# akhilmurthy/spacedrive

Hardware: AMD Instinct MI355X
Metric: cas_id files/sec + BLAKE3 GB/s hashed (node) at 1/2/4/8 MI355X (higher is better)
Workload: dtype u32

## Files before the change

### include/sdcas.h

```cpp
#ifndef SDCAS_H
#define SDCAS_H

#include <stddef.h>
#include <stdint.h>

#ifdef __cplusplus
extern "C" {
#endif

#define SDCAS_OK 0
#define SDCAS_E_NO_DEVICE (-1)
#define SDCAS_E_INVALID (-2)
#define SDCAS_E_OOM (-3)
#define SDCAS_E_HIP (-4)
#define SDCAS_E_CAPACITY (-5)
#define SDCAS_E_CANCELLED (-6)

#define SDCAS_STATUS_UNEXPECTED_EOF 100001
#define SDCAS_STATUS_CANCELLED 125

#define SDCAS_MAX_BATCH 0x7FFFFFFF

#define SDCAS_SAMPLE_COUNT 4
#define SDCAS_SAMPLE_SIZE 10240
// ... 284 lines not shown
int sdcas_dev_dedup_combine_async(sdcas_ctx *ctx, const uint64_t *d_keys, const uint8_t *d_has_key,
                                  const int32_t *d_status, const uint64_t *d_ids, size_t n, uint32_t world,
                                  uint64_t *d_rec, uint32_t *d_slot, uint32_t *d_starts, void *stream);
int sdcas_dev_dedup_resolve(sdcas_ctx *ctx, const uint64_t *d_frec, size_t nf, const uint64_t *d_erec,
                            size_t ne, int64_t *d_result, void *stream);
int sdcas_dev_dedup_apply(sdcas_ctx *ctx, const uint64_t *d_ids, const uint32_t *d_slot, size_t n,
                          const int64_t *d_result, size_t chunk_size, const uint64_t *d_plan, int64_t *d_link,
                          uint64_t *d_counts, void *stream);
int sdcas_dev_dedup_combine_buckets(sdcas_ctx *ctx, const uint64_t *d_keys, const uint8_t *d_has_key,
                                    const int32_t *d_status, const uint64_t *d_ids, size_t n, uint32_t world,
                                    size_t cap, uint64_t *d_send, uint32_t *d_slot, int64_t *d_counts,
                                    uint32_t *d_overflow, void *stream);
int sdcas_dev_dedup_resolve_buckets(sdcas_ctx *ctx, const uint64_t *d_frec, size_t fcap, const int64_t *d_fcounts,
                                    const uint64_t *d_erec, size_t ecap, const int64_t *d_ecounts, uint32_t world,
                                    int64_t *d_result, void *stream);
int sdcas_dev_dedup_local(sdcas_ctx *ctx, const uint64_t *d_keys, const uint8_t *d_has_key,
                          const int32_t *d_status, const uint64_t *d_ids, size_t n, const uint64_t *d_ekeys,
                          const uint64_t *d_eids, size_t ne, size_t chunk_size, uint64_t n_total,
                          uint64_t max_steps, uint32_t more, int64_t *d_link, uint64_t *d_counts,
                          uint64_t *d_plan_header, void *stream);

typedef struct sdcas_node sdcas_node;
int sdcas_node_init(const int32_t *devices, size_t n_devices, const sdcas_options *opts, sdcas_node **out_node);
void sdcas_node_destroy(sdcas_node *node);
const char *sdcas_node_last_error(const sdcas_node *node);
size_t sdcas_node_size(const sdcas_node *node);
int sdcas_node_uses_rccl(const sdcas_node *node);
int sdcas_node_set_progress(sdcas_node *node, sdcas_progress_fn progress, void *user, const volatile int32_t *cancel);
int sdcas_node_cas_ids(sdcas_node *node, const char *const *paths, const uint64_t *sizes, size_t n,
                       uint64_t *out_keys, int32_t *out_status);
// ... 15 lines not shown
```

### spacedrive_amd/csrc/b3_batch.h

```cpp
#pragma once
#include <hip/hip_runtime.h>
#include <stddef.h>
#include <stdint.h>

namespace sdcas {

constexpr uint32_t kTile = 1024;
constexpr uint32_t kWG = 512;
constexpr uint32_t kSmallTile = 128;
constexpr uint64_t kSmallSlots = 1ull << 14;
constexpr int kSmallVariant = 84;
constexpr uint32_t kSortTotalsWords = 256;
constexpr uint32_t kSortPerWG = 4096;
inline size_t sort_key_words(size_t max_msgs) { return kSortTotalsWords + 256 * (max_msgs / kSortPerWG + 1); }

struct BatchWorkspace {
  uint64_t* S = nullptr;
  uint32_t* tile_first = nullptr;
  uint64_t* total = nullptr;
  uint32_t* nodes = nullptr;
  void* scan_tmp = nullptr;
  size_t scan_tmp_bytes = 0;
  uint32_t cap_msgs = 0;
  uint64_t cap_chunks = 0;
  uint64_t cap_slots = 0;
  int variant = -1;
  uint64_t small_slots = kSmallSlots;
  int small_variant = kSmallVariant;
  uint64_t cap_small_tiles = 0;
// ... 79 lines not shown
```

### spacedrive_amd/csrc/b3_batch.hip

```cpp
#include <hip/hip_runtime.h>

#include <atomic>
#ifdef SDCAS_ABLATIONS
#include <hipcub/hipcub.hpp>
#endif
#include <stdint.h>
#include <cstdio>
#include <cstring>

#include "b3_device.h"
#include "b3_batch.h"
#include "b3_tree.h"

namespace sdcas {

using namespace b3d;

constexpr int kMaxStack = 64;
constexpr int kMaxStackBig = 64;


template <uint32_t TILE = kTile>
__global__ void k_tile_first(const uint64_t* __restrict__ lens, const uint64_t* __restrict__ S, uint32_t n,
                             uint64_t cap_chunks, uint32_t* __restrict__ tile_first, uint64_t* __restrict__ total) {
// ... 928 lines not shown
                       dim3(kFinishQWG), 0, st, lens, n, S, tile_first, total, cap_slots, nodes, perm, out32,
                       out_keys);
  else
    hipLaunchKernelGGL(k_finish_t<TILE>, dim3((uint32_t)((tiles + kFinishWG - 1) / kFinishWG)), dim3(kFinishWG), 0,
                       st, lens, n, S, tile_first, total, cap_slots, nodes, perm, out32, out_keys);
}

#ifdef SDCAS_ABLATIONS
#include "b3_ablate_kernels.inc"
#endif

constexpr uint32_t kShapeBins = 256;
constexpr uint32_t kScatterPerWG = 4096;
constexpr uint32_t kScatterR = kScatterPerWG / 256;
constexpr uint32_t kShapeManyChunks = 15 << 4;
static_assert(kSortTotalsWords == kShapeBins && kSortPerWG == kScatterPerWG, "ws.sort_keys layout");

__device__ __forceinline__ uint32_t shape_key(uint64_t L) {
  const uint64_t C = chunk_count(L);
  const uint64_t last = L - (C - 1) * CHUNK_LEN;
  const uint32_t blocks = last == 0 ? 1u : (uint32_t)((last + BLOCK_LEN - 1) / BLOCK_LEN);
  return ((uint32_t)min<uint64_t>(C, 15) << 4) | (blocks - 1);
}

__global__ void __launch_bounds__(256) k_shape_hist(const uint64_t* __restrict__ lens, uint32_t n,
                                                    uint32_t* __restrict__ wcnt) {
  __shared__ uint32_t h[kShapeBins];
  const uint32_t t = threadIdx.x;
  h[t] = 0;
  __syncthreads();
  const uint64_t lo = (uint64_t)blockIdx.x * kScatterPerWG;
  uint64_t L[kScatterR];
#pragma unroll
  for (uint32_t r = 0; r < kScatterR; ++r) {
    const uint64_t i = lo + r * 256 + t;
    L[r] = i < n ? lens[i] : 0;
  }
#pragma unroll
  for (uint32_t r = 0; r < kScatterR; ++r)
    if (lo + r * 256 + t < n) atomicAdd(&h[shape_key(L[r])], 1u);
  __syncthreads();
  wcnt[(uint64_t)t * gridDim.x + blockIdx.x] = h[t];
}

__global__ void __launch_bounds__(256) k_shape_bins(uint32_t* __restrict__ wcnt, uint32_t nwg,
                                                    uint32_t* __restrict__ totals) {
  __shared__ uint32_t ws[4];
  __shared__ uint32_t carry;
  const uint32_t t = threadIdx.x, lane = t & 63, wave = t >> 6;
  uint32_t* col = wcnt + (uint64_t)blockIdx.x * nwg;
  if (t == 0) carry = 0;
  __syncthreads();
  for (uint32_t base = 0; base < nwg; base += 256) {
    const uint32_t i = base + t;
    const uint32_t v = i < nwg ? col[i] : 0u;
    uint32_t inc = v;
#pragma unroll
    for (uint32_t d = 1; d < 64; d <<= 1) {
      const uint32_t x = __shfl_up(inc, d);
      if (lane >= d) inc += x;
    }
    if (lane == 63) ws[wave] = inc;
    __syncthreads();
    uint32_t before = carry;
    for (uint32_t w = 0; w < wave; ++w) before += ws[w];
    if (i < nwg) col[i] = before + inc - v;
    __syncthreads();
    if (t == 255) carry = before + inc;
    __syncthreads();
  }
  if (t == 0) totals[blockIdx.x] = carry;
}

__global__ void __launch_bounds__(256) k_shape_scatter(const uint64_t* __restrict__ offs,
                                                       const uint64_t* __restrict__ lens, uint32_t n,
                                                       const uint32_t* __restrict__ totals,
                                                       const uint32_t* __restrict__ wstart,
                                                       uint32_t* __restrict__ perm, uint64_t* __restrict__ soffs,
                                                       uint64_t* __restrict__ slens) {
  __shared__ uint32_t gstart[kShapeBins], lstart[kShapeBins], h[kShapeBins];
  __shared__ uint16_t order[kScatterPerWG];
  __shared__ uint8_t keyof[kScatterPerWG];
  __shared__ uint32_t few_chunks;
  const uint32_t t = threadIdx.x;
  const uint32_t bin_count = totals[t];
  gstart[t] = bin_count;
  h[t] = 0;
  __syncthreads();
  for (uint32_t d = 1; d < kShapeBins; d <<= 1) {
    const uint32_t v = t >= d ? gstart[t - d] : 0u;
    __syncthreads();
    gstart[t] += v;
    __syncthreads();
  }
  if (t == kShapeManyChunks - 1) few_chunks = gstart[t];
  const uint32_t excl = gstart[t] - bin_count;
  __syncthreads();
  gstart[t] = excl;
  const uint32_t lo = blockIdx.x * kScatterPerWG, hi = min(n, lo + kScatterPerWG), m = hi - lo;
  if ((uint64_t)(n - few_chunks) * 10 > (uint64_t)n * 6) {
    uint64_t o[kScatterR], l[kScatterR];
#pragma unroll
    for (uint32_t r = 0; r < kScatterR; ++r) {
      const uint32_t k = t + r * 256;
      o[r] = k < m ? offs[lo + k] : 0;
      l[r] = k < m ? lens[lo + k] : 0;
    }
#pragma unroll
    for (uint32_t r = 0; r < kScatterR; ++r) {
      const uint32_t k = t + r * 256;
      if (k >= m) continue;
      perm[lo + k] = lo + k;
      soffs[lo + k] = o[r];
      slens[lo + k] = l[r];
    }
    return;
  }
  {
    uint64_t l[kScatterR];
#pragma unroll
    for (uint32_t r = 0; r < kScatterR; ++r) {
      const uint32_t k = t + r * 256;
      l[r] = k < m ? lens[lo + k] : 0;
    }
#pragma unroll
    for (uint32_t r = 0; r < kScatterR; ++r) {
      const uint32_t k = t + r * 256;
      if (k >= m) continue;
      const uint32_t key = shape_key(l[r]);
      keyof[k] = (uint8_t)key;
      atomicAdd(&h[key], 1u);
    }
  }
  __syncthreads();
  const uint32_t cnt = h[t];
  gstart[t] += wstart[(uint64_t)t * gridDim.x + blockIdx.x];
  lstart[t] = cnt;
  __syncthreads();
  for (uint32_t d = 1; d < kShapeBins; d <<= 1) {
    const uint32_t v = t >= d ? lstart[t - d] : 0u;
    __syncthreads();
    lstart[t] += v;
    __syncthreads();
  }
  lstart[t] -= cnt;
  h[t] = 0;
  __syncthreads();
  for (uint32_t k = t; k < m; k += 256) {
    const uint32_t key = keyof[k];
    order[lstart[key] + atomicAdd(&h[key], 1u)] = (uint16_t)k;
  }
  __syncthreads();
  uint32_t kk[kScatterR];
  uint64_t o[kScatterR], l[kScatterR];
#pragma unroll
  for (uint32_t r = 0; r < kScatterR; ++r) {
    const uint32_t p = t + r * 256;
    kk[r] = p < m ? order[p] : 0u;
    o[r] = p < m ? offs[lo + kk[r]] : 0;
    l[r] = p < m ? lens[lo + kk[r]] : 0;
  }
#pragma unroll
  for (uint32_t r = 0; r < kScatterR; ++r) {
    const uint32_t p = t + r * 256;
    if (p >= m) continue;
    const uint32_t key = keyof[kk[r]];
    const uint32_t pos = gstart[key] + (p - lstart[key]);
    perm[pos] = lo + kk[r];
    soffs[pos] = o[r];
    slens[pos] = l[r];
  }
}



template <int PF, int DIRECT, int ROT, int TOP, int DEFER>
__device__ __forceinline__ void piece_pass(const uint8_t* __restrict__ blob, const PieceDesc* __restrict__ pieces,
                                           uint32_t npieces, uint32_t* __restrict__ file_nodes,
                                           uint32_t* __restrict__ l4) {
  __shared__ uint32_t cvs[kTile][8];
  __shared__ uint16_t task[kTile / 2];
  __shared__ uint32_t ntask[16];
  const uint32_t tid = threadIdx.x;
  for (uint32_t pi = blockIdx.x; pi < npieces; pi += gridDim.x) {
    const PieceDesc pd = pieces[pi];
// ... 564 lines not shown

hipError_t finish_crossing(uint64_t tiles, const uint64_t* lens, uint32_t n, const uint64_t* S,
                           const uint32_t* tile_first, const uint64_t* total, uint64_t cap_slots,
                           const uint32_t* nodes, uint8_t* out32, uint64_t* out_keys, hipStream_t st) {
  launch_finish<kTile>(tiles, st, lens, n, S, tile_first, total, cap_slots, nodes, nullptr, out32, out_keys);
  return hipGetLastError();
}

hipError_t batch_hash(const BatchWorkspace& ws, const uint8_t* blob, const uint64_t* offs, const uint64_t* lens,
                      uint32_t n, uint8_t* out32, uint64_t* out_keys, hipStream_t st, uint64_t max_chunks,
                      hipEvent_t ev0, hipEvent_t ev1, const BatchPlan* plan) {
  if (n == 0) return hipSuccess;
  if (n > ws.cap_msgs) return hipErrorInvalidValue;
  [[maybe_unused]] hipError_t e;
  const uint32_t* perm = nullptr;
  if (ws.sort && n >= kSortMinMsgs && ws.perm) {
    const uint32_t nwg = (n + kScatterPerWG - 1) / kScatterPerWG;
    uint32_t* totals = ws.sort_keys;
    uint32_t* wcnt = ws.sort_keys + kSortTotalsWords;
    hipLaunchKernelGGL(k_shape_hist, dim3(nwg), dim3(256), 0, st, lens, n, wcnt);
    hipLaunchKernelGGL(k_shape_bins, dim3(kShapeBins), dim3(256), 0, st, wcnt, nwg, totals);
    hipLaunchKernelGGL(k_shape_scatter, dim3(nwg), dim3(256), 0, st, offs, lens, n, totals, wcnt, ws.perm, ws.soffs,
                       ws.slens);
    offs = ws.soffs;
    lens = ws.slens;
    perm = ws.perm;
  }
  const bool forced = leaf_variant_available(ws.variant) || leaf_variant_forced();
  int v = leaf_variant_available(ws.variant) ? ws.variant : leaf_variant();
  bool quad = false;
#ifdef SDCAS_ABLATIONS
  quad = kLeafVariants[v].quad && (perm || n == 1);
  if (kLeafVariants[v].quad && !quad) v = kDefaultLeafVariant;
#endif
  const uint64_t slots =
      max_chunks ? std::min<uint64_t>(ws.cap_slots, max_chunks + (quad ? 3ull * n + 8 : 0)) : ws.cap_slots;
  if (!forced && !quad && slots <= ws.small_slots && slots / kSmallTile + 2 <= ws.cap_small_tiles)
    v = leaf_variant_available(ws.small_variant) && kLeafVariants[ws.small_variant].tile == kSmallTile ? ws.small_variant
                                                                                                        : kSmallVariant;
  if (kLeafVariants[v].tile == kSmallTile && slots / kSmallTile + 2 > ws.cap_small_tiles) v = kDefaultLeafVariant;
  const uint32_t tile = kLeafVariants[v].tile;
  const bool planned = plan && !perm && !quad && plan->tile == tile;
  uint64_t* const S = planned ? const_cast<uint64_t*>(plan->S) : ws.S;
  uint32_t* const tile_first = planned ? const_cast<uint32_t*>(plan->tile_first) : ws.tile_first;
  uint64_t* const total = planned ? plan->total : ws.total;
  size_t tmp = ws.scan_tmp_bytes;
  if (planned) {
  } else if (quad) {
#ifdef SDCAS_ABLATIONS
    QuadIt qit(hipcub::CountingInputIterator<uint32_t>(0), QuadSlotsOp{lens, n});
    if ((e = hipcub::DeviceScan::ExclusiveSum(ws.scan_tmp, tmp, qit, ws.S, (int)n, st))) return e;
    hipLaunchKernelGGL(k_tile_first_q, dim3((n + 255) / 256), dim3(256), 0, st, lens, ws.S, n, ws.cap_slots,
                       ws.tile_first, ws.total);
#endif
  } else {
    const uint32_t nb = (n + kPlanPer - 1) / kPlanPer;
    if ((size_t)(nb + 1) * sizeof(uint64_t) > tmp) return hipErrorInvalidValue;
    uint64_t* bsum = static_cast<uint64_t*>(ws.scan_tmp);
    hipLaunchKernelGGL(k_plan_sums, dim3(nb), dim3(kPlanWG), 0, st, lens, n, bsum);
    hipLaunchKernelGGL(k_plan_scan, dim3(1), dim3(1024), 0, st, bsum, nb, ws.total);
    if (tile == kSmallTile)
      hipLaunchKernelGGL(k_plan_write<kSmallTile>, dim3(nb), dim3(kPlanWG), 0, st, lens, n, bsum, ws.cap_slots, ws.S,
                         ws.tile_first);
    else
      hipLaunchKernelGGL(k_plan_write<kTile>, dim3(nb), dim3(kPlanWG), 0, st, lens, n, bsum, ws.cap_slots, ws.S,
                         ws.tile_first);
  }
  if (ev0) (void)hipEventRecord(ev0, st);
  {
// ... 177 lines not shown
```

### spacedrive_amd/csrc/dist_dedup.h

```cpp
#pragma once
#include <hip/hip_runtime.h>
#include <stddef.h>
#include <stdint.h>

namespace sdcas {

constexpr uint32_t kSlotNoKey = 0xFFFFFFFFu;
constexpr uint32_t kSlotDropped = 0xFFFFFFFEu;

__host__ __device__ inline uint32_t dd_owner(uint64_t key, uint32_t world) {
  return (uint32_t)(((key >> 52) * (uint64_t)world) >> 12);
}

struct DistWs {
  template <class T>
  struct Buf {
    T* p = nullptr;
    size_t cap = 0;
    hipError_t ensure(size_t n) {
      if (n <= cap) return hipSuccess;
      if (p) (void)hipFree(p);
      p = nullptr;
      cap = 0;
      size_t want = n < 16 ? 16 : n;
// ... 60 lines not shown

hipError_t dd_resolve_buckets(DistWs& w, const uint64_t* frec, uint32_t fcap, const int64_t* fcounts,
                              const uint64_t* erec, uint32_t ecap, const int64_t* ecounts, uint32_t world,
                              int64_t* result, hipStream_t st);

hipError_t dd_resolve(DistWs& w, const uint64_t* frec, uint32_t nf, const uint64_t* erec, uint32_t ne,
                      int64_t* result, hipStream_t st);

hipError_t dd_apply(DistWs& w, const uint64_t* ids, const uint32_t* slot, uint32_t n, const int64_t* result,
                    uint64_t chunk_size, const uint64_t* plan, int64_t* link, unsigned long long* counts,
                    hipStream_t st);

hipError_t dd_local(DistWs& w, const uint64_t* keys, const uint8_t* has_key, const int32_t* status,
                    const uint64_t* ids, uint32_t n, const uint64_t* ekeys, const uint64_t* eids, uint32_t ne,
                    uint64_t chunk_size, const StepWindow& win, int64_t* link, unsigned long long* counts,
                    hipStream_t st);

}
```

### spacedrive_amd/csrc/dist_dedup.hip

```cpp
#include <hip/hip_runtime.h>

#include <algorithm>
#include <atomic>
#include <cstdlib>
#include <cstring>

#include "dist_dedup.h"
#include "wg_scan.h"

namespace sdcas {

namespace {

constexpr uint32_t TB = 256;
constexpr int64_t kLinkDeferred = INT64_MIN + 1;
inline uint32_t blocks(uint32_t n) { return (n + TB - 1) / TB; }
constexpr uint32_t kIdxEmpty = 0xFFFFFFFFu;
constexpr uint32_t kCountShards = 64;


constexpr uint32_t kRrBuckets = 4096;
constexpr uint32_t kRrWords = 2 + (kRrBuckets + 2) / 2;
constexpr uint32_t kRrMin = 64;

// ... 1174 lines not shown
    const int kind = h == kSlotDropped ? kFileDropped : h == kSlotNoKey ? kFileNoKey : kFileKeyed;
    int64_t r = 0;
    if (kind == kFileKeyed) {
      const uint32_t f = tab[h];
      const uint64_t e = ebase != kIdxEmpty ? (f >= ebase ? emin[f - ebase] : ~0ull) : emin ? emin[h] : ~0ull;
      r = e != ~0ull ? -(int64_t)e - 1 : (int64_t)(f == i ? ids[i] : ids[f]);
    }
    link[i] = step_link(kind, (int64_t)ids[i], r, cs, pv, c, l);
  }
  add_counts(c, l, sc, counts);
}



__global__ void k_local_clear(uint4* __restrict__ tab, uint64_t tab_q, uint4* __restrict__ em, uint64_t em_q,
                              uint32_t* __restrict__ cnt, uint32_t nt, uint32_t* __restrict__ flag) {
  const uint4 ones = make_uint4(~0u, ~0u, ~0u, ~0u);
  const uint64_t stride = (uint64_t)gridDim.x * blockDim.x;
  const uint64_t t0 = (uint64_t)blockIdx.x * blockDim.x + threadIdx.x;
  for (uint64_t q = t0; q < tab_q; q += stride) tab[q] = ones;
  for (uint64_t q = t0; q < em_q; q += stride) em[q] = ones;
  for (uint64_t q = t0; q < nt; q += stride) cnt[q] = 0;
  if (flag && t0 == 0) *flag = 0;
}

template <uint32_t R>
__global__ void __launch_bounds__(TB) k_solo_apply_r(const uint64_t* __restrict__ ids,
                                                     const uint32_t* __restrict__ pos, uint32_t n,
                                                     const uint32_t* __restrict__ tab,
                                                     const uint64_t* __restrict__ emin, uint64_t cs,
                                                     const uint64_t* __restrict__ plan, int64_t* __restrict__ link,
                                                     unsigned long long* __restrict__ shard,
                                                     const uint32_t* __restrict__ noncontig, uint32_t ebase,
                                                     const uint64_t* __restrict__ ridx) {
  __shared__ unsigned long long sc[2];
  if (threadIdx.x < 2) sc[threadIdx.x] = 0;
  __syncthreads();
  const PlanView pv = plan_view(plan, ridx);
// ... 145 lines not shown
}

static bool exist_min_by_entry() {
  const char* v = getenv("SDCAS_EXIST_MIN");
  return !(v && strcmp(v, "slot") == 0);
}

static bool plain_probe() {
  const char* v = getenv("SDCAS_PROBE");
  return v && strcmp(v, "plain") == 0;
}

static hipError_t local_fused(DistWs& w, const uint64_t* keys, const uint8_t* has_key, const int32_t* status,
                              const uint64_t* ids, uint32_t n, const uint64_t* ekeys, const uint64_t* eids,
                              uint32_t ne, uint64_t cs, const StepWindow& win, int64_t* link,
                              unsigned long long* counts, uint64_t cap, hipStream_t st) {
  hipError_t e;
  const uint32_t nt = (n + kStayTile - 1) / kStayTile;
  const bool stays = has_key || status;
  const uint32_t mask = (uint32_t)(cap - 1);
  const uint32_t shift = 64u - (uint32_t)__builtin_ctzll(cap);
  const uint32_t ar = apply_files_per_thread();
  const bool sharded = ar && counts;
  const bool contig = ar && contig_ordinals() && n > 0;
  const bool entry = ne && exist_min_by_entry();
  const uint32_t sticky = entry ? n : kIdxEmpty;
  if ((e = w.tmin.ensure(cap / 2 + 1)) || (e = w.tpos.ensure(n)) ||
      (ne && (e = w.tkey.ensure(entry ? (uint64_t)ne + 2 : cap + 1))) ||
      (e = w.stay_cnt.ensure(nt + stay_groups(nt) + 1)) || (stays && (e = w.stay_sorted.ensure(n))) ||
      (sharded && (e = shard_counts(w, st))) ||
      (contig && (e = w.flag.ensure(1))))
    return e;
  auto* tab = reinterpret_cast<uint32_t*>(w.tmin.p);
  auto* em = ne ? reinterpret_cast<unsigned long long*>(w.tkey.p) : nullptr;
  const uint64_t tab_q = cap / 4, em_q = !ne ? 0 : entry ? ((uint64_t)ne + 1) / 2 : cap / 2;
  const uint32_t cg = (uint32_t)std::min<uint64_t>((tab_q + em_q + TB - 1) / TB, 2048);
  hipLaunchKernelGGL(k_local_clear, dim3(cg), dim3(TB), 0, st, reinterpret_cast<uint4*>(tab), tab_q,
                     reinterpret_cast<uint4*>(em), em_q, w.stay_cnt.p, stays ? nt + stay_groups(nt) : 0u,
                     contig ? w.flag.p : (uint32_t*)nullptr);
  if (ne)
    hipLaunchKernelGGL(k_solo_insert_idx, dim3(blocks(ne)), dim3(TB), 0, st, keys, ekeys, n, (const uint8_t*)nullptr,
                       (const int32_t*)nullptr, eids, ne, n, tab, em, mask, shift, (uint32_t*)nullptr,
                       (uint32_t*)nullptr, (uint32_t*)nullptr, sticky);
  hipLaunchKernelGGL(k_solo_insert_idx, dim3(blocks(n)), dim3(TB), 0, st, keys, ekeys, n, has_key, status,
                     contig ? ids : (const uint64_t*)nullptr, n, 0u, tab, (unsigned long long*)nullptr, mask, shift,
                     w.tpos.p, stays ? w.stay_cnt.p : (uint32_t*)nullptr, contig ? w.flag.p : (uint32_t*)nullptr,
                     sticky, plain_probe() ? 1u : 0u);
  if (stays)
    hipLaunchKernelGGL(k_stays_write_t<kStayTile>, dim3(nt), dim3(TB), 0, st, has_key, status, n, w.stay_cnt.p,
                       w.stay_idx.p, ids, w.stay_sorted.p);
  hipLaunchKernelGGL(k_plan_walk, dim3(1), dim3(64), 0, st, (const uint64_t*)w.stay_sorted.p, (const uint32_t*)nullptr,
                     ids, stays ? n : 0u, (const uint32_t*)nullptr, win.n_total ? win.n_total : (uint64_t)n, cs,
                     win.max_steps, win.more, w.plan.p, stays ? w.stay_cnt.p + nt : (const uint32_t*)nullptr,
                     stay_groups(nt));
// ... 149 lines not shown
                         w.stay_sorted.p);
      tcnt = w.stay_cnt.p;
    }
    sorted = w.stay_sorted.p;
  }
  hipLaunchKernelGGL(k_plan_walk, dim3(1), dim3(64), 0, st, sorted, (const uint32_t*)nullptr,
                     (const uint64_t*)nullptr, n_stays, (const uint32_t*)nullptr, win.n_total, cs, win.max_steps,
                     win.more, plan, tcnt, ntiles);
  if (n_stays >= kRrMin && (e = rr_index(w, plan, st))) return e;
  return hipGetLastError();
}

hipError_t dd_local(DistWs& w, const uint64_t* keys, const uint8_t* has_key, const int32_t* status,
                    const uint64_t* ids, uint32_t n, const uint64_t* ekeys, const uint64_t* eids, uint32_t ne,
                    uint64_t chunk_size, const StepWindow& win, int64_t* link, unsigned long long* counts,
                    hipStream_t st) {
  hipError_t e;
  if (chunk_size == 0) chunk_size = 100;
  if ((e = w.nstay.ensure(1)) || (e = w.plan.ensure(kPlanHeader + (uint64_t)n + 1))) return e;
  const DedupTable table = dedup_table();
  if (n && table == kTableIdx) {
    const uint64_t cap = local_cap((uint64_t)n + ne);
    if (cap > (1ull << 31)) return hipErrorInvalidValue;
    return local_fused(w, keys, has_key, status, ids, n, ekeys, eids, ne, chunk_size, win, link, counts, cap, st);
  }
  if (n && (has_key || status)) {
    if ((e = select_stays(w, has_key, status, n, st))) return e;
  } else if ((e = hipMemsetAsync(w.nstay.p, 0, sizeof(uint32_t), st))) {
    return e;
  }
  hipLaunchKernelGGL(k_plan_walk, dim3(1), dim3(64), 0, st, (const uint64_t*)nullptr, w.stay_idx.p, ids, n,
                     w.nstay.p, win.n_total ? win.n_total : (uint64_t)n, chunk_size, win.max_steps, win.more, w.plan.p);
  if (n == 0) return hipGetLastError();
  const uint64_t cap = local_cap((uint64_t)n + ne);
  if (cap > (1ull << 31)) return hipErrorInvalidValue;
  if (table == kTableIdx4) {
    const uint32_t mask = (uint32_t)(cap - 1);
    const uint32_t shift = 64u - (uint32_t)__builtin_ctzll(cap);
    if ((e = w.tmin.ensure(cap / 2 + 1)) || (e = w.tpos.ensure(n)) || (ne && (e = w.tkey.ensure(cap + 1)))) return e;
    auto* tab = reinterpret_cast<uint32_t*>(w.tmin.p);
// ... 130 lines not shown
```

### spacedrive_amd/csrc/sdcas_api.hip

```cpp
#include <fcntl.h>
#include <hip/hip_runtime.h>
#include <sys/mman.h>
#include <sys/stat.h>
#include <unistd.h>

#include <algorithm>
#include <atomic>
#include <cerrno>
#include <cstdarg>
#include <cstdio>
#include <cstring>
#include <mutex>
#include <string>
#include <thread>
#include <chrono>
#include <memory>
#include <vector>

#include "../../include/sdcas.h"
#include "../../include/sdcas_bench.h"
#include "../host/cas_io.hpp"
#include "b3_batch.h"
#include "confirm.h"
#include "dupsets.h"
// ... 1644 lines not shown
  if (!c || (n && (!keys || !has_key || !out_link)) || (n_existing && !existing_keys)) return SDCAS_E_INVALID;
  if (!dedup_fits(n, n_existing))
    return c->fail(SDCAS_E_CAPACITY, "dedup of %zu files + %zu Objects exceeds 2^30", n, n_existing);
  PathCall call(c);
  if (call.rc) return call.rc;
  if (chunk_size == 0) chunk_size = SDCAS_IDENTIFIER_CHUNK_SIZE;
  hipError_t e;
  hipStream_t st = c->stream;
  if ((e = c->dd_keys.ensure(n)) || (e = c->dd_has.ensure(n)) || (e = c->dd_link.ensure(n)) ||
      (status && (e = c->dd_status.ensure(n))) || (e = c->dd_ekeys.ensure(n_existing + 1)) ||
      (e = c->dd_counts.ensure(2)))
    return c->hip_fail(e, "dedup buffers");
  if ((e = hipMemcpyAsync(c->dd_keys.p, keys, 8 * n, hipMemcpyHostToDevice, st)) ||
      (e = hipMemcpyAsync(c->dd_has.p, has_key, n, hipMemcpyHostToDevice, st)) ||
      (status && (e = hipMemcpyAsync(c->dd_status.p, status, 4 * n, hipMemcpyHostToDevice, st))) ||
      (n_existing && (e = hipMemcpyAsync(c->dd_ekeys.p, existing_keys, 8 * n_existing, hipMemcpyHostToDevice, st))) ||
      (e = hipMemsetAsync(c->dd_counts.p, 0, 2 * sizeof(unsigned long long), st)))
    return c->hip_fail(e, "dedup H2D");
  if ((e = iota(c->dd_ids, std::max(n, n_existing), st))) return c->hip_fail(e, "dedup ids");
  StepWindow sw;
  sw.n_total = n;
  sw.max_steps = win ? win->max_steps : 0;
  sw.more = win ? win->more : 0;
  if ((e = dd_local(c->dist, c->dd_keys.p, c->dd_has.p, status ? c->dd_status.p : nullptr, c->dd_ids.p, (uint32_t)n,
                    c->dd_ekeys.p, c->dd_ids.p, (uint32_t)n_existing, chunk_size, sw, c->dd_link.p, c->dd_counts.p,
                    st)))
    return c->hip_fail(e, "dedup");
  unsigned long long cnt[2] = {0, 0};
  uint64_t hdr[kPlanHeader] = {};
  if ((n && (e = hipMemcpyAsync(out_link, c->dd_link.p, 8 * n, hipMemcpyDeviceToHost, st))) ||
      (e = hipMemcpyAsync(cnt, c->dd_counts.p, sizeof cnt, hipMemcpyDeviceToHost, st)) ||
      (e = hipMemcpyAsync(hdr, c->dist.plan.p, sizeof hdr, hipMemcpyDeviceToHost, st)))
    return c->hip_fail(e, "dedup D2H");
  if ((e = hipStreamSynchronize(st))) return c->hip_fail(e, "dedup sync");
  if (out_created) *out_created = (int64_t)cnt[0];
  if (out_linked) *out_linked = (int64_t)cnt[1];
  if (win) {
    win->steps = hdr[kPlanSteps];
    win->rows = hdr[kPlanRows];
    win->rereads = hdr[kPlanRereadsRun];
  }
// ... 3 lines not shown
int sdcas_dedup(sdcas_ctx* c, const uint64_t* keys, const uint8_t* has_key, const int32_t* status, size_t n,
                size_t chunk_size, const uint64_t* existing_keys, size_t n_existing, int64_t* out_link,
                int64_t* out_created, int64_t* out_linked) {
  return sdcas_dedup_window(c, keys, has_key, status, n, chunk_size, existing_keys, n_existing, nullptr, out_link,
                            out_created, out_linked);
}

int sdcas_dev_dedup(sdcas_ctx* c, const uint64_t* d_keys, const uint8_t* d_has_key, const int32_t* d_status,
                    size_t n, size_t chunk_size, int64_t* d_out_link, uint64_t* d_counts, void* stream) {
  if (!c || (n && (!d_keys || !d_has_key || !d_out_link))) return SDCAS_E_INVALID;
  if (!dedup_fits(n, 0)) return c->fail(SDCAS_E_CAPACITY, "dev_dedup of %zu files exceeds 2^30", n);
  DevCall call(c, stream);
  if (call.rc) return call.rc;
  if (chunk_size == 0) chunk_size = SDCAS_IDENTIFIER_CHUNK_SIZE;
  hipError_t e;
  if (d_counts && (e = hipMemsetAsync(d_counts, 0, 2 * sizeof(uint64_t), call.st))) return c->hip_fail(e, "counts");
  if ((e = iota(c->dd_ids, n, call.st))) return c->hip_fail(e, "dev_dedup ids");
  e = dd_local(c->dist, d_keys, d_has_key, d_status, c->dd_ids.p, (uint32_t)n, nullptr, nullptr, 0, chunk_size,
               StepWindow{}, d_out_link, (unsigned long long*)d_counts, call.st);
  return e ? c->hip_fail(e, "dev_dedup") : SDCAS_OK;
}


static int confirm_ws(sdcas_ctx* c, size_t n, hipStream_t st) {
  const size_t need = (size_t)confirm_ws_words(n);
  if (need <= c->cf_ws.cap) return SDCAS_OK;
  hipError_t e = c->scratch_sync();
  if (!e) e = hipStreamSynchronize(st);
  if (!e) e = c->cf_ws.ensure(need);
  return e ? c->hip_fail(e, "confirm workspace") : SDCAS_OK;
}

int sdcas_dev_confirm_duplicates(sdcas_ctx* c, const uint64_t* d_keys, const uint8_t* d_digests32,
                                 const uint8_t* d_valid, size_t n, int64_t* d_out_rep, int64_t* d_out_key_rep,
// ... 1070 lines not shown
                                    world, d_result, call.st);
  return e ? c->hip_fail(e, "dedup_resolve_buckets") : SDCAS_OK;
}

int sdcas_dev_dedup_local(sdcas_ctx* c, const uint64_t* d_keys, const uint8_t* d_has_key, const int32_t* d_status,
                          const uint64_t* d_ids, size_t n, const uint64_t* d_ekeys, const uint64_t* d_eids, size_t ne,
                          size_t chunk_size, uint64_t n_total, uint64_t max_steps, uint32_t more, int64_t* d_link,
                          uint64_t* d_counts, uint64_t* d_plan_header, void* stream) {
  if (!c || (n && (!d_keys || !d_ids || !d_link)) || (ne && (!d_ekeys || !d_eids))) return SDCAS_E_INVALID;
  if (!dedup_fits(n, ne)) return c->fail(SDCAS_E_CAPACITY, "dedup_local: %zu + %zu records exceed 2^30", n, ne);
  DevCall call(c, stream);
  if (call.rc) return call.rc;
  StepWindow sw;
  sw.n_total = n_total;
  sw.max_steps = max_steps;
  sw.more = more;
  hipError_t e = dd_local(c->dist, d_keys, d_has_key, d_status, d_ids, (uint32_t)n, d_ekeys, d_eids, (uint32_t)ne,
                          chunk_size ? chunk_size : SDCAS_IDENTIFIER_CHUNK_SIZE, sw, d_link,
                          (unsigned long long*)d_counts, call.st);
  if (!e && d_plan_header)
    e = hipMemcpyAsync(d_plan_header, c->dist.plan.p, 8 * kPlanHeader, hipMemcpyDeviceToDevice, call.st);
  return e ? c->hip_fail(e, "dedup_local") : SDCAS_OK;
}

int sdcas_dev_dedup_stays(sdcas_ctx* c, const uint8_t* d_has_key, const int32_t* d_status, const uint64_t* d_ids,
                          size_t n, size_t cap, uint64_t* d_stays, int64_t* d_count, void* stream) {
  if (!c || (n && (d_has_key || d_status) && !d_ids) || (cap && !d_stays)) return SDCAS_E_INVALID;
  if (n > SDCAS_MAX_BATCH || cap > SDCAS_MAX_BATCH)
    return c->fail(SDCAS_E_CAPACITY, "dedup_stays: %zu files / %zu entries exceed 2^31 - 1", n, cap);
  DevCall call(c, stream);
  if (call.rc) return call.rc;
  hipError_t e = dd_stays(c->dist, d_has_key, d_status, d_ids, (uint32_t)n, (uint32_t)cap, d_stays, d_count, call.st);
  return e ? c->hip_fail(e, "dedup_stays") : SDCAS_OK;
}
// ... 171 lines not shown
```

### spacedrive_amd/dist_dedup.py

```python
from __future__ import annotations

import ctypes
import os
import sys
import time

import numpy as np
import torch
import torch.distributed as dist

from . import _native as N


class DeviceStages:

    def __init__(self, engine, device=None, same_stream=False):
        self.eng = engine
        self.device = torch.device("cuda", torch.cuda.current_device() if device is None else device)
        self.stream = torch.cuda.Stream(self.device)
        self.same_stream = same_stream

    def _current(self):
        cur = torch.cuda.current_stream(self.device)
        return cur if self.same_stream and cur.cuda_stream else None
# ... 31 lines not shown

    def resolve(self, frec, erec):
        nf, ne = int(frec.shape[0]), int(erec.shape[0])
        result = torch.empty(max(nf, 1), dtype=torch.int64, device=frec.device)
        p = lambda t: t.data_ptr() if t.numel() else None
        rc = self.eng.L.sdcas_dev_dedup_resolve(self.eng.ctx, p(frec), nf, p(erec), ne, p(result),
                                                self._enter())
        self._leave(frec, erec, result)
        self.eng._check(rc, "sdcas_dev_dedup_resolve")
        return result[:nf]

    def local(self, keys, has_key, status, ids, chunk_size, existing_keys=None, existing_ids=None, n_total=0,
              max_steps=0, more=False, header=None):
        n = int(ids.numel())
        link = torch.empty(max(n, 1), dtype=torch.int64, device=ids.device)
        counts = torch.zeros(2, dtype=torch.int64, device=ids.device)
        ne = int(existing_keys.numel()) if existing_keys is not None else 0
        p = lambda t: t.data_ptr() if t is not None and t.numel() else None
        rc = self.eng.L.sdcas_dev_dedup_local(self.eng.ctx, p(keys), p(has_key), p(status), p(ids), n,
                                              p(existing_keys) if ne else None, p(existing_ids) if ne else None,
                                              ne, int(chunk_size), int(n_total), int(max_steps), int(bool(more)),
                                              p(link), counts.data_ptr(), p(header), self._enter())
        self._leave(keys, has_key, status, ids, existing_keys, existing_ids, link, counts, header)
        self.eng._check(rc, "sdcas_dev_dedup_local")
        return link[:n], counts

    def stays(self, has_key, status, ids, cap):
        n = int(ids.numel())
        out = torch.empty(max(cap, 1), dtype=torch.int64, device=ids.device)
        count = torch.empty(1, dtype=torch.int64, device=ids.device)
        p = lambda t: t.data_ptr() if t is not None and t.numel() else None
        rc = self.eng.L.sdcas_dev_dedup_stays(self.eng.ctx, p(has_key), p(status), p(ids), n, int(cap), p(out),
                                              count.data_ptr(), self._enter())
        self._leave(has_key, status, ids, out, count)
        self.eng._check(rc, "sdcas_dev_dedup_stays")
        return out[:cap], count
# ... 336 lines not shown
```

Baseline: 65.16 million.

## Fuse slot planning into shape-sort scatter and fold counts clearing into dedup clear

```diff
diff --git a/include/sdcas.h b/include/sdcas.h
--- a/include/sdcas.h
+++ b/include/sdcas.h
@@ -322,6 +322,7 @@
 int sdcas_dev_dedup_resolve_buckets(sdcas_ctx *ctx, const uint64_t *d_frec, size_t fcap, const int64_t *d_fcounts,
                                     const uint64_t *d_erec, size_t ecap, const int64_t *d_ecounts, uint32_t world,
                                     int64_t *d_result, void *stream);
+#define SDCAS_DEDUP_COUNTS_OVERWRITE 2u
 int sdcas_dev_dedup_local(sdcas_ctx *ctx, const uint64_t *d_keys, const uint8_t *d_has_key,
                           const int32_t *d_status, const uint64_t *d_ids, size_t n, const uint64_t *d_ekeys,
                           const uint64_t *d_eids, size_t ne, size_t chunk_size, uint64_t n_total,
diff --git a/spacedrive_amd/csrc/b3_batch.h b/spacedrive_amd/csrc/b3_batch.h
--- a/spacedrive_amd/csrc/b3_batch.h
+++ b/spacedrive_amd/csrc/b3_batch.h
@@ -11,8 +11,13 @@
 constexpr uint64_t kSmallSlots = 1ull << 14;
 constexpr int kSmallVariant = 84;
 constexpr uint32_t kSortTotalsWords = 256;
+constexpr uint32_t kSortChunksWord = 256;
+constexpr uint32_t kSortHeadWords = 768;
 constexpr uint32_t kSortPerWG = 4096;
-inline size_t sort_key_words(size_t max_msgs) { return kSortTotalsWords + 256 * (max_msgs / kSortPerWG + 1); }
+constexpr uint32_t kSortManyBins = 16;
+inline size_t sort_key_words(size_t max_msgs) {
+  return kSortHeadWords + (256 + 2 * kSortManyBins) * (max_msgs / kSortPerWG + 1);
+}
 
 struct BatchWorkspace {
   uint64_t* S = nullptr;
diff --git a/spacedrive_amd/csrc/b3_batch.hip b/spacedrive_amd/csrc/b3_batch.hip
--- a/spacedrive_amd/csrc/b3_batch.hip
+++ b/spacedrive_amd/csrc/b3_batch.hip
@@ -966,7 +966,10 @@
 constexpr uint32_t kScatterPerWG = 4096;
 constexpr uint32_t kScatterR = kScatterPerWG / 256;
 constexpr uint32_t kShapeManyChunks = 15 << 4;
-static_assert(kSortTotalsWords == kShapeBins && kSortPerWG == kScatterPerWG, "ws.sort_keys layout");
+static_assert(kSortTotalsWords == kShapeBins && kSortChunksWord == kSortTotalsWords &&
+                  kSortHeadWords == kSortChunksWord + 2 * kShapeBins && kSortPerWG == kScatterPerWG &&
+                  kSortManyBins == kShapeBins - kShapeManyChunks,
+              "ws.sort_keys layout");
 
 __device__ __forceinline__ uint32_t shape_key(uint64_t L) {
   const uint64_t C = chunk_count(L);
@@ -975,11 +978,25 @@
   return ((uint32_t)min<uint64_t>(C, 15) << 4) | (blocks - 1);
 }
 
+__device__ __forceinline__ uint64_t wg256_incl_scan(uint64_t v, uint64_t* wv, uint32_t lane, uint32_t wave) {
+  uint64_t inc = wave_incl_scan(v, lane);
+  if (lane == 63) wv[wave] = inc;
+  __syncthreads();
+#pragma unroll
+  for (uint32_t w = 0; w < 3; ++w)
+    if (w < wave) inc += wv[w];
+  __syncthreads();
+  return inc;
+}
+
 __global__ void __launch_bounds__(256) k_shape_hist(const uint64_t* __restrict__ lens, uint32_t n,
-                                                    uint32_t* __restrict__ wcnt) {
+                                                    uint32_t* __restrict__ wcnt,
+                                                    unsigned long long* __restrict__ wsum) {
   __shared__ uint32_t h[kShapeBins];
+  __shared__ unsigned long long hs[kSortManyBins];
   const uint32_t t = threadIdx.x;
   h[t] = 0;
+  if (t < kSortManyBins) hs[t] = 0;
   __syncthreads();
   const uint64_t lo = (uint64_t)blockIdx.x * kScatterPerWG;
   uint64_t L[kScatterR];
@@ -990,65 +1007,151 @@
   }
 #pragma unroll
   for (uint32_t r = 0; r < kScatterR; ++r)
-    if (lo + r * 256 + t < n) atomicAdd(&h[shape_key(L[r])], 1u);
+    if (lo + r * 256 + t < n) {
+      const uint32_t key = shape_key(L[r]);
+      atomicAdd(&h[key], 1u);
+      if (key >= kShapeManyChunks) atomicAdd(&hs[key - kShapeManyChunks], (unsigned long long)chunk_count(L[r]));
+    }
   __syncthreads();
   wcnt[(uint64_t)t * gridDim.x + blockIdx.x] = h[t];
-}
-
-__global__ void __launch_bounds__(256) k_shape_bins(uint32_t* __restrict__ wcnt, uint32_t nwg,
-                                                    uint32_t* __restrict__ totals) {
+  if (t < kSortManyBins) wsum[(uint64_t)t * gridDim.x + blockIdx.x] = hs[t];
+}
+
+__global__ void __launch_bounds__(256) k_shape_bins(uint32_t* __restrict__ wcnt,
+                                                    unsigned long long* __restrict__ wsum, uint32_t nwg,
+                                                    uint32_t* __restrict__ head) {
   __shared__ uint32_t ws[4];
+  __shared__ uint64_t wl[4];
   __shared__ uint32_t carry;
+  __shared__ uint64_t lcarry;
   const uint32_t t = threadIdx.x, lane = t & 63, wave = t >> 6;
-  uint32_t* col = wcnt + (uint64_t)blockIdx.x * nwg;
-  if (t == 0) carry = 0;
+  const uint32_t b = blockIdx.x;
+  const bool many = b >= kShapeManyChunks;
+  uint32_t* col = wcnt + (uint64_t)b * nwg;
+  unsigned long long* lcol = many ? wsum + (uint64_t)(b - kShapeManyChunks) * nwg : nullptr;
+  if (t == 0) {
+    carry = 0;
+    lcarry = 0;
+  }
   __syncthreads();
   for (uint32_t base = 0; base < nwg; base += 256) {
     const uint32_t i = base + t;
     const uint32_t v = i < nwg ? col[i] : 0u;
+    const uint64_t lv = many && i < nwg ? lcol[i] : 0;
     uint32_t inc = v;
 #pragma unroll
     for (uint32_t d = 1; d < 64; d <<= 1) {
       const uint32_t x = __shfl_up(inc, d);
       if (lane >= d) inc += x;
     }
-    if (lane == 63) ws[wave] = inc;
+    const uint64_t linc = many ? wave_incl_scan(lv, lane) : 0;
+    if (lane == 63) {
+      ws[wave] = inc;
+      wl[wave] = linc;
+    }
     __syncthreads();
     uint32_t before = carry;
-    for (uint32_t w = 0; w < wave; ++w) before += ws[w];
-    if (i < nwg) col[i] = before + inc - v;
+    uint64_t lbefore = lcarry;
+    for (uint32_t w = 0; w < wave; ++w) {
+      before += ws[w];
+      lbefore += wl[w];
+    }
+    if (i < nwg) {
+      col[i] = before + inc - v;
+      if (many) lcol[i] = lbefore + linc - lv;
+    }
     __syncthreads();
-    if (t == 255) carry = before + inc;
+    if (t == 255) {
+      carry = before + inc;
+      lcarry = lbefore + linc;
+    }
     __syncthreads();
   }
-  if (t == 0) totals[blockIdx.x] = carry;
-}
-
-__global__ void __launch_bounds__(256) k_shape_scatter(const uint64_t* __restrict__ offs,
+  if (t == 0) {
+    head[b] = carry;
+    reinterpret_cast<uint64_t*>(head + kSortChunksWord)[b] = many ? lcarry : (uint64_t)(b >> 4) * carry;
+  }
+}
+
+
+__device__ __forceinline__ void scatter_prefix(uint32_t (&s0)[kScatterR], uint32_t (*part)[4], uint32_t lane,
+                                               uint32_t wave) {
+#pragma unroll
+  for (uint32_t r = 0; r < kScatterR; ++r) {
+    uint32_t inc = s0[r];
+#pragma unroll
+    for (uint32_t d = 1; d < 64; d <<= 1) {
+      const uint32_t x = __shfl_up(inc, d);
+      if (lane >= d) inc += x;
+    }
+    s0[r] = inc - s0[r];
+    if (lane == 63) part[r][wave] = inc;
+  }
+  __syncthreads();
+  uint32_t run = 0;
+#pragma unroll
+  for (uint32_t r = 0; r < kScatterR; ++r) {
+    uint32_t all = 0;
+#pragma unroll
+    for (uint32_t w = 0; w < 4; ++w) {
+      const uint32_t v = part[r][w];
+      if (w < wave) s0[r] += v;
+      all += v;
+    }
+    s0[r] += run;
+    run += all;
+  }
+}
+
+__device__ __forceinline__ void write_plan(uint64_t s0, uint64_t C, uint32_t pos, uint32_t tile_shift,
+                                           uint64_t cap_slots, uint64_t* __restrict__ S,
+                                           uint32_t* __restrict__ tile_first) {
+  S[pos] = s0;
+  const uint64_t tile = 1ull << tile_shift;
+  for (uint64_t q = (s0 + tile - 1) >> tile_shift; (q << tile_shift) < s0 + C && (q << tile_shift) < cap_slots; ++q)
+    tile_first[q] = pos;
+}
+
+__global__ void __launch_bounds__(256) __attribute__((amdgpu_waves_per_eu(3, 3)))
+k_shape_scatter(const uint64_t* __restrict__ offs,
                                                        const uint64_t* __restrict__ lens, uint32_t n,
-                                                       const uint32_t* __restrict__ totals,
+                                                       const uint32_t* __restrict__ head,
                                                        const uint32_t* __restrict__ wstart,
+                                                       const unsigned long long* __restrict__ wsum,
                                                        uint32_t* __restrict__ perm, uint64_t* __restrict__ soffs,
-                                                       uint64_t* __restrict__ slens) {
+                                                       uint64_t* __restrict__ slens, uint64_t* __restrict__ S,
+                                                       uint32_t* __restrict__ tile_first,
+                                                       uint64_t* __restrict__ total, uint64_t cap_slots,
+                                                       uint32_t tile_shift) {
   __shared__ uint32_t gstart[kShapeBins], lstart[kShapeBins], h[kShapeBins];
+  __shared__ uint64_t sstart[kShapeBins];
+  __shared__ uint32_t part[kScatterR][4];
+  __shared__ uint64_t wv[4];
+  __shared__ uint32_t few_chunks;
+  __shared__ uint64_t before_wg;
   __shared__ uint16_t order[kScatterPerWG];
   __shared__ uint8_t keyof[kScatterPerWG];
-  __shared__ uint32_t few_chunks;
-  const uint32_t t = threadIdx.x;
-  const uint32_t bin_count = totals[t];
-  gstart[t] = bin_count;
+  const uint32_t t = threadIdx.x, lane = t & 63, wave = t >> 6;
+  const uint32_t bin_count = head[t];
+  const uint64_t bin_chunks = reinterpret_cast<const uint64_t*>(head + kSortChunksWord)[t];
+  const uint32_t wfirst = wstart[(uint64_t)t * gridDim.x + blockIdx.x];
+  const uint64_t cbefore = t < kShapeManyChunks
+                               ? (uint64_t)(t >> 4) * wfirst
+                               : (uint64_t)wsum[(uint64_t)(t - kShapeManyChunks) * gridDim.x + blockIdx.x];
+  const uint32_t upto = (uint32_t)wg256_incl_scan(bin_count, wv, lane, wave);
+  const uint64_t slots = wg256_incl_scan(bin_chunks, wv, lane, wave);
+  const uint64_t wg_before = wg256_incl_scan(cbefore, wv, lane, wave);
+  gstart[t] = upto - bin_count + wfirst;
   h[t] = 0;
+  if (t == kShapeManyChunks - 1) few_chunks = upto;
+  if (t == kShapeBins - 1) {
+    before_wg = wg_before;
+    if (S && blockIdx.x == 0) {
+      total[0] = slots;
+      total[2] = 0;
+    }
+  }
   __syncthreads();
-  for (uint32_t d = 1; d < kShapeBins; d <<= 1) {
-    const uint32_t v = t >= d ? gstart[t - d] : 0u;
-    __syncthreads();
-    gstart[t] += v;
-    __syncthreads();
-  }
-  if (t == kShapeManyChunks - 1) few_chunks = gstart[t];
-  const uint32_t excl = gstart[t] - bin_count;
-  __syncthreads();
-  gstart[t] = excl;
   const uint32_t lo = blockIdx.x * kScatterPerWG, hi = min(n, lo + kScatterPerWG), m = hi - lo;
   if ((uint64_t)(n - few_chunks) * 10 > (uint64_t)n * 6) {
     uint64_t o[kScatterR], l[kScatterR];
@@ -1066,8 +1169,28 @@
       soffs[lo + k] = o[r];
       slens[lo + k] = l[r];
     }
+    if (!S) return;
+    uint32_t s0[kScatterR];
+#pragma unroll
+    for (uint32_t r = 0; r < kScatterR; ++r) s0[r] = t + r * 256 < m ? (uint32_t)chunk_count(l[r]) : 0u;
+    scatter_prefix(s0, part, lane, wave);
+#pragma unroll
+    for (uint32_t r = 0; r < kScatterR; ++r) {
+      const uint32_t k = t + r * 256;
+      if (k < m) write_plan(before_wg + s0[r], chunk_count(l[r]), lo + k, tile_shift, cap_slots, S, tile_first);
+    }
     return;
   }
+  uint64_t many_chunks = 0;
+  if (t < kSortManyBins) {
+    const uint64_t* col = reinterpret_cast<const uint64_t*>(wsum) + (uint64_t)t * gridDim.x;
+    const uint64_t mine = col[blockIdx.x];
+    const uint64_t next = blockIdx.x + 1 < gridDim.x
+                              ? col[blockIdx.x + 1]
+                              : reinterpret_cast<const uint64_t*>(head + kSortChunksWord)[kShapeManyChunks + t];
+    many_chunks = next - mine;
+  }
+  sstart[t] = many_chunks;
   {
     uint64_t l[kScatterR];
 #pragma unroll
@@ -1086,16 +1209,11 @@
   }
   __syncthreads();
   const uint32_t cnt = h[t];
-  gstart[t] += wstart[(uint64_t)t * gridDim.x + blockIdx.x];
-  lstart[t] = cnt;
-  __syncthreads();
-  for (uint32_t d = 1; d < kShapeBins; d <<= 1) {
-    const uint32_t v = t >= d ? lstart[t - d] : 0u;
-    __syncthreads();
-    lstart[t] += v;
-    __syncthreads();
-  }
-  lstart[t] -= cnt;
+  const uint64_t csum = t < kShapeManyChunks ? (uint64_t)(t >> 4) * cnt : sstart[t - kShapeManyChunks];
+  const uint32_t lupto = (uint32_t)wg256_incl_scan(cnt, wv, lane, wave);
+  const uint64_t cupto = wg256_incl_scan(csum, wv, lane, wave);
+  lstart[t] = lupto - cnt;
+  sstart[t] = slots - bin_chunks + cbefore - (cupto - csum);
   h[t] = 0;
   __syncthreads();
   for (uint32_t k = t; k < m; k += 256) {
@@ -1121,6 +1239,19 @@
     perm[pos] = lo + kk[r];
     soffs[pos] = o[r];
     slens[pos] = l[r];
+  }
+  if (!S) return;
+  uint32_t s0[kScatterR];
+#pragma unroll
+  for (uint32_t r = 0; r < kScatterR; ++r) s0[r] = t + r * 256 < m ? (uint32_t)chunk_count(l[r]) : 0u;
+  scatter_prefix(s0, part, lane, wave);
+#pragma unroll
+  for (uint32_t r = 0; r < kScatterR; ++r) {
+    const uint32_t p = t + r * 256;
+    if (p >= m) continue;
+    const uint32_t key = keyof[kk[r]];
+    write_plan(sstart[key] + s0[r], chunk_count(l[r]), gstart[key] + (p - lstart[key]), tile_shift, cap_slots, S,
+               tile_first);
   }
 }
 
@@ -1715,23 +1846,12 @@
   if (n > ws.cap_msgs) return hipErrorInvalidValue;
   [[maybe_unused]] hipError_t e;
   const uint32_t* perm = nullptr;
-  if (ws.sort && n >= kSortMinMsgs && ws.perm) {
-    const uint32_t nwg = (n + kScatterPerWG - 1) / kScatterPerWG;
-    uint32_t* totals = ws.sort_keys;
-    uint32_t* wcnt = ws.sort_keys + kSortTotalsWords;
-    hipLaunchKernelGGL(k_shape_hist, dim3(nwg), dim3(256), 0, st, lens, n, wcnt);
-    hipLaunchKernelGGL(k_shape_bins, dim3(kShapeBins), dim3(256), 0, st, wcnt, nwg, totals);
-    hipLaunchKernelGGL(k_shape_scatter, dim3(nwg), dim3(256), 0, st, offs, lens, n, totals, wcnt, ws.perm, ws.soffs,
-                       ws.slens);
-    offs = ws.soffs;
-    lens = ws.slens;
-    perm = ws.perm;
-  }
+  const bool sorted = ws.sort && n >= kSortMinMsgs && ws.perm;
   const bool forced = leaf_variant_available(ws.variant) || leaf_variant_forced();
   int v = leaf_variant_available(ws.variant) ? ws.variant : leaf_variant();
   bool quad = false;
 #ifdef SDCAS_ABLATIONS
-  quad = kLeafVariants[v].quad && (perm || n == 1);
+  quad = kLeafVariants[v].quad && (sorted || n == 1);
   if (kLeafVariants[v].quad && !quad) v = kDefaultLeafVariant;
 #endif
   const uint64_t slots =
@@ -1741,6 +1861,23 @@
                                                                                                         : kSmallVariant;
   if (kLeafVariants[v].tile == kSmallTile && slots / kSmallTile + 2 > ws.cap_small_tiles) v = kDefaultLeafVariant;
   const uint32_t tile = kLeafVariants[v].tile;
+  const bool fused = sorted && !quad && ws.cap_slots < (1ull << 32);
+  if (sorted) {
+    const uint32_t nwg = (n + kScatterPerWG - 1) / kScatterPerWG;
+    uint32_t* head = ws.sort_keys;
+    uint32_t* wcnt = ws.sort_keys + kSortHeadWords;
+    auto* wsum = reinterpret_cast<unsigned long long*>(wcnt + (size_t)kShapeBins * nwg);
+    if (fused && (tile & (tile - 1))) return hipErrorInvalidValue;
+    hipLaunchKernelGGL(k_shape_hist, dim3(nwg), dim3(256), 0, st, lens, n, wcnt, wsum);
+    hipLaunchKernelGGL(k_shape_bins, dim3(kShapeBins), dim3(256), 0, st, wcnt, wsum, nwg, head);
+    hipLaunchKernelGGL(k_shape_scatter, dim3(nwg), dim3(256), 0, st, offs, lens, n, (const uint32_t*)head,
+                       (const uint32_t*)wcnt, (const unsigned long long*)wsum, ws.perm, ws.soffs, ws.slens,
+                       fused ? ws.S : (uint64_t*)nullptr, ws.tile_first, ws.total, ws.cap_slots,
+                       (uint32_t)__builtin_ctz(tile));
+    offs = ws.soffs;
+    lens = ws.slens;
+    perm = ws.perm;
+  }
   const bool planned = plan && !perm && !quad && plan->tile == tile;
   uint64_t* const S = planned ? const_cast<uint64_t*>(plan->S) : ws.S;
   uint32_t* const tile_first = planned ? const_cast<uint32_t*>(plan->tile_first) : ws.tile_first;
@@ -1754,6 +1891,7 @@
     hipLaunchKernelGGL(k_tile_first_q, dim3((n + 255) / 256), dim3(256), 0, st, lens, ws.S, n, ws.cap_slots,
                        ws.tile_first, ws.total);
 #endif
+  } else if (fused) {
   } else {
     const uint32_t nb = (n + kPlanPer - 1) / kPlanPer;
     if ((size_t)(nb + 1) * sizeof(uint64_t) > tmp) return hipErrorInvalidValue;
diff --git a/spacedrive_amd/csrc/dist_dedup.h b/spacedrive_amd/csrc/dist_dedup.h
--- a/spacedrive_amd/csrc/dist_dedup.h
+++ b/spacedrive_amd/csrc/dist_dedup.h
@@ -98,6 +98,6 @@
 hipError_t dd_local(DistWs& w, const uint64_t* keys, const uint8_t* has_key, const int32_t* status,
                     const uint64_t* ids, uint32_t n, const uint64_t* ekeys, const uint64_t* eids, uint32_t ne,
                     uint64_t chunk_size, const StepWindow& win, int64_t* link, unsigned long long* counts,
-                    hipStream_t st);
+                    hipStream_t st, bool counts_overwrite = false);
 
 }
diff --git a/spacedrive_amd/csrc/dist_dedup.hip b/spacedrive_amd/csrc/dist_dedup.hip
--- a/spacedrive_amd/csrc/dist_dedup.hip
+++ b/spacedrive_amd/csrc/dist_dedup.hip
@@ -1212,7 +1212,8 @@
 
 
 __global__ void k_local_clear(uint4* __restrict__ tab, uint64_t tab_q, uint4* __restrict__ em, uint64_t em_q,
-                              uint32_t* __restrict__ cnt, uint32_t nt, uint32_t* __restrict__ flag) {
+                              uint32_t* __restrict__ cnt, uint32_t nt, uint32_t* __restrict__ flag,
+                              unsigned long long* __restrict__ counts) {
   const uint4 ones = make_uint4(~0u, ~0u, ~0u, ~0u);
   const uint64_t stride = (uint64_t)gridDim.x * blockDim.x;
   const uint64_t t0 = (uint64_t)blockIdx.x * blockDim.x + threadIdx.x;
@@ -1220,6 +1221,7 @@
   for (uint64_t q = t0; q < em_q; q += stride) em[q] = ones;
   for (uint64_t q = t0; q < nt; q += stride) cnt[q] = 0;
   if (flag && t0 == 0) *flag = 0;
+  if (counts && t0 == 0) counts[0] = counts[1] = 0;
 }
 
 template <uint32_t R>
@@ -1395,7 +1397,7 @@
 static hipError_t local_fused(DistWs& w, const uint64_t* keys, const uint8_t* has_key, const int32_t* status,
                               const uint64_t* ids, uint32_t n, const uint64_t* ekeys, const uint64_t* eids,
                               uint32_t ne, uint64_t cs, const StepWindow& win, int64_t* link,
-                              unsigned long long* counts, uint64_t cap, hipStream_t st) {
+                              unsigned long long* counts, bool counts_overwrite, uint64_t cap, hipStream_t st) {
   hipError_t e;
   const uint32_t nt = (n + kStayTile - 1) / kStayTile;
   const bool stays = has_key || status;
@@ -1418,7 +1420,7 @@
   const uint32_t cg = (uint32_t)std::min<uint64_t>((tab_q + em_q + TB - 1) / TB, 2048);
   hipLaunchKernelGGL(k_local_clear, dim3(cg), dim3(TB), 0, st, reinterpret_cast<uint4*>(tab), tab_q,
                      reinterpret_cast<uint4*>(em), em_q, w.stay_cnt.p, stays ? nt + stay_groups(nt) : 0u,
-                     contig ? w.flag.p : (uint32_t*)nullptr);
+                     contig ? w.flag.p : (uint32_t*)nullptr, counts_overwrite ? counts : (unsigned long long*)nullptr);
   if (ne)
     hipLaunchKernelGGL(k_solo_insert_idx, dim3(blocks(ne)), dim3(TB), 0, st, keys, ekeys, n, (const uint8_t*)nullptr,
                        (const int32_t*)nullptr, eids, ne, n, tab, em, mask, shift, (uint32_t*)nullptr,
@@ -1598,16 +1600,19 @@
 hipError_t dd_local(DistWs& w, const uint64_t* keys, const uint8_t* has_key, const int32_t* status,
                     const uint64_t* ids, uint32_t n, const uint64_t* ekeys, const uint64_t* eids, uint32_t ne,
                     uint64_t chunk_size, const StepWindow& win, int64_t* link, unsigned long long* counts,
-                    hipStream_t st) {
+                    hipStream_t st, bool counts_overwrite) {
   hipError_t e;
   if (chunk_size == 0) chunk_size = 100;
+  counts_overwrite = counts_overwrite && counts;
   if ((e = w.nstay.ensure(1)) || (e = w.plan.ensure(kPlanHeader + (uint64_t)n + 1))) return e;
   const DedupTable table = dedup_table();
   if (n && table == kTableIdx) {
     const uint64_t cap = local_cap((uint64_t)n + ne);
     if (cap > (1ull << 31)) return hipErrorInvalidValue;
-    return local_fused(w, keys, has_key, status, ids, n, ekeys, eids, ne, chunk_size, win, link, counts, cap, st);
-  }
+    return local_fused(w, keys, has_key, status, ids, n, ekeys, eids, ne, chunk_size, win, link, counts,
+                       counts_overwrite, cap, st);
+  }
+  if (counts_overwrite && (e = hipMemsetAsync(counts, 0, 2 * sizeof(unsigned long long), st))) return e;
   if (n && (has_key || status)) {
     if ((e = select_stays(w, has_key, status, n, st))) return e;
   } else if ((e = hipMemsetAsync(w.nstay.p, 0, sizeof(uint32_t), st))) {
diff --git a/spacedrive_amd/csrc/sdcas_api.hip b/spacedrive_amd/csrc/sdcas_api.hip
--- a/spacedrive_amd/csrc/sdcas_api.hip
+++ b/spacedrive_amd/csrc/sdcas_api.hip
@@ -1682,8 +1682,7 @@
   if ((e = hipMemcpyAsync(c->dd_keys.p, keys, 8 * n, hipMemcpyHostToDevice, st)) ||
       (e = hipMemcpyAsync(c->dd_has.p, has_key, n, hipMemcpyHostToDevice, st)) ||
       (status && (e = hipMemcpyAsync(c->dd_status.p, status, 4 * n, hipMemcpyHostToDevice, st))) ||
-      (n_existing && (e = hipMemcpyAsync(c->dd_ekeys.p, existing_keys, 8 * n_existing, hipMemcpyHostToDevice, st))) ||
-      (e = hipMemsetAsync(c->dd_counts.p, 0, 2 * sizeof(unsigned long long), st)))
+      (n_existing && (e = hipMemcpyAsync(c->dd_ekeys.p, existing_keys, 8 * n_existing, hipMemcpyHostToDevice, st))))
     return c->hip_fail(e, "dedup H2D");
   if ((e = iota(c->dd_ids, std::max(n, n_existing), st))) return c->hip_fail(e, "dedup ids");
   StepWindow sw;
@@ -1692,7 +1691,7 @@
   sw.more = win ? win->more : 0;
   if ((e = dd_local(c->dist, c->dd_keys.p, c->dd_has.p, status ? c->dd_status.p : nullptr, c->dd_ids.p, (uint32_t)n,
                     c->dd_ekeys.p, c->dd_ids.p, (uint32_t)n_existing, chunk_size, sw, c->dd_link.p, c->dd_counts.p,
-                    st)))
+                    st, true)))
     return c->hip_fail(e, "dedup");
   unsigned long long cnt[2] = {0, 0};
   uint64_t hdr[kPlanHeader] = {};
@@ -1726,10 +1725,9 @@
   if (call.rc) return call.rc;
   if (chunk_size == 0) chunk_size = SDCAS_IDENTIFIER_CHUNK_SIZE;
   hipError_t e;
-  if (d_counts && (e = hipMemsetAsync(d_counts, 0, 2 * sizeof(uint64_t), call.st))) return c->hip_fail(e, "counts");
   if ((e = iota(c->dd_ids, n, call.st))) return c->hip_fail(e, "dev_dedup ids");
   e = dd_local(c->dist, d_keys, d_has_key, d_status, c->dd_ids.p, (uint32_t)n, nullptr, nullptr, 0, chunk_size,
-               StepWindow{}, d_out_link, (unsigned long long*)d_counts, call.st);
+               StepWindow{}, d_out_link, (unsigned long long*)d_counts, call.st, true);
   return e ? c->hip_fail(e, "dev_dedup") : SDCAS_OK;
 }
 
@@ -2830,10 +2828,10 @@
   StepWindow sw;
   sw.n_total = n_total;
   sw.max_steps = max_steps;
-  sw.more = more;
+  sw.more = more & 1u;
   hipError_t e = dd_local(c->dist, d_keys, d_has_key, d_status, d_ids, (uint32_t)n, d_ekeys, d_eids, (uint32_t)ne,
                           chunk_size ? chunk_size : SDCAS_IDENTIFIER_CHUNK_SIZE, sw, d_link,
-                          (unsigned long long*)d_counts, call.st);
+                          (unsigned long long*)d_counts, call.st, (more & SDCAS_DEDUP_COUNTS_OVERWRITE) != 0);
   if (!e && d_plan_header)
     e = hipMemcpyAsync(d_plan_header, c->dist.plan.p, 8 * kPlanHeader, hipMemcpyDeviceToDevice, call.st);
   return e ? c->hip_fail(e, "dedup_local") : SDCAS_OK;
diff --git a/spacedrive_amd/dist_dedup.py b/spacedrive_amd/dist_dedup.py
--- a/spacedrive_amd/dist_dedup.py
+++ b/spacedrive_amd/dist_dedup.py
@@ -69,12 +69,12 @@
               max_steps=0, more=False, header=None):
         n = int(ids.numel())
         link = torch.empty(max(n, 1), dtype=torch.int64, device=ids.device)
-        counts = torch.zeros(2, dtype=torch.int64, device=ids.device)
+        counts = torch.empty(2, dtype=torch.int64, device=ids.device)
         ne = int(existing_keys.numel()) if existing_keys is not None else 0
         p = lambda t: t.data_ptr() if t is not None and t.numel() else None
         rc = self.eng.L.sdcas_dev_dedup_local(self.eng.ctx, p(keys), p(has_key), p(status), p(ids), n,
                                               p(existing_keys) if ne else None, p(existing_ids) if ne else None,
-                                              ne, int(chunk_size), int(n_total), int(max_steps), int(bool(more)),
+                                              ne, int(chunk_size), int(n_total), int(max_steps), int(bool(more)) | 2,
                                               p(link), counts.data_ptr(), p(header), self._enter())
         self._leave(keys, has_key, status, ids, existing_keys, existing_ids, link, counts, header)
         self.eng._check(rc, "sdcas_dev_dedup_local")
```

Result: no change. 65.16 million, median of 2 (+0.0%).
